# MaaniGhaffari/cvo-rgbd

Hardware: AMD Instinct MI355X
Metric: frame-pair registrations/sec (higher is better)
Workload: dtype f32; 1 GPU; BASELINE configs[1] shape: 64 distinct synthetic 10000x10000 RGB-D cloud pairs (xyz + 5-dim colour) per align_many call, cvo align() to convergence, clouds resident in HBM; points_fixed=10000, points_moving=10000, mode=cvo, batch=64

## Files before the change

cvo-rgbd_amd/capi.py:

```python
import collections
import ctypes as C
import os

import numpy as np

_HERE = os.path.dirname(os.path.abspath(__file__))
LIB_PATH = os.path.join(_HERE, "csrc", "libcvo_hip.so")
_LIB = None

MODE_CVO, MODE_ACVO, MODE_MATLAB = 0, 1, 2
FEAT_COLMAJOR, FEAT_ROWMAJOR = 0, 1

SYMBOLS = [
    "cvo_hip_error_string", "cvo_hip_last_error", "cvo_hip_device_count",
    "cvo_hip_default_params", "cvo_hip_init_state", "cvo_hip_create", "cvo_hip_destroy",
    "cvo_hip_set_params", "cvo_hip_set_fixed", "cvo_hip_set_moving",
    "cvo_hip_set_fixed_device", "cvo_hip_set_moving_device",
    "cvo_hip_swap_moving_to_fixed", "cvo_hip_set_pcd_many", "cvo_hip_get_device_cloud", "cvo_hip_range_filter_grid_average", "cvo_hip_set_shard", "cvo_hip_shard_range",
    "cvo_hip_comm_unique_id", "cvo_hip_comm_init", "cvo_hip_set_allreduce",
    "cvo_hip_mailbox_create", "cvo_hip_mailbox_connect",
    "cvo_hip_transform_pcd", "cvo_hip_flow", "cvo_hip_step_coeffs", "cvo_hip_pose_hessian", "cvo_hip_pose_score",
    "cvo_hip_pose_score_many", "cvo_hip_pose_scan", "cvo_hip_pose_matches", "cvo_hip_pick_step",
    "cvo_hip_exp_se3", "cvo_hip_dist_se3", "cvo_hip_align", "cvo_hip_align_many",
    "cvo_hip_function_inner_product", "cvo_hip_function_inner_product_clouds",
    "cvo_hip_engine_profiling", "cvo_hip_get_engine_profile", "cvo_hip_get_engine_flow_trace", "cvo_hip_get_wave_load", "cvo_hip_set_graph_capture", "cvo_hip_set_profiling", "cvo_hip_get_profile", "cvo_hip_get_graph_stats", "cvo_hip_get_run_stats", "cvo_hip_get_list_stats", "cvo_hip_get_run_clocks", "cvo_hip_get_mirror_retries", "cvo_hip_synchronize",
    "cvo_hip_set_option", "cvo_hip_get_option",
]


class Params(C.Structure):
    _fields_ = [
        ("mode", C.c_int32), ("max_iter", C.c_int32),
        ("ell_init", C.c_float), ("ell_min", C.c_float), ("ell_max_init", C.c_float),
        ("sigma", C.c_float), ("sp_thres", C.c_float), ("c_sp_thres", C.c_float),
        ("c", C.c_float), ("d", C.c_float), ("c_ell", C.c_float), ("c_sigma", C.c_float),
        ("min_step", C.c_float), ("eps", C.c_float), ("eps_2", C.c_float), ("color_scale", C.c_float),
        ("dl_step", C.c_double),
    ]


class State(C.Structure):
    _fields_ = [
        ("R", C.c_float * 9), ("T", C.c_float * 3),
        ("ell", C.c_float), ("ell_max", C.c_float),
        ("transform", C.c_float * 16), ("prev_transform", C.c_float * 16),
        ("accum_transform", C.c_float * 16),
        ("iter", C.c_int32), ("pad_", C.c_int32),
    ]
# ... 150 lines not shown
    L.cvo_hip_transform_pcd.argtypes = [vp, fp, fp]
    L.cvo_hip_flow.argtypes = [vp, C.c_float, dp]
    L.cvo_hip_step_coeffs.argtypes = [vp, fp, fp, C.c_float, dp]
    L.cvo_hip_pose_hessian.argtypes = [vp, fp, fp, C.c_float, C.POINTER(PoseHessianC)]
    L.cvo_hip_pose_score.argtypes = [vp, fp, fp, C.c_float, C.POINTER(PoseScoreC)]
    L.cvo_hip_pose_score_many.argtypes = [C.POINTER(vp), fp, fp, fp, C.POINTER(PoseScoreC), C.c_int]
    L.cvo_hip_pose_scan.argtypes = [vp, fp, fp, C.c_int, C.c_float, C.POINTER(PoseScanEntryC), C.POINTER(PoseScanC)]
    L.cvo_hip_pose_matches.argtypes = [vp, fp, fp, C.c_float, C.POINTER(PointMatchesC), C.POINTER(PointMatchesC),
                                       C.POINTER(PoseMatchesC)]
    L.cvo_hip_pick_step.argtypes = [dp, C.c_float, fp]
    L.cvo_hip_exp_se3.argtypes = [fp, fp, C.c_float, fp, fp]
    L.cvo_hip_dist_se3.argtypes = [fp, fp, C.c_float, fp]
    L.cvo_hip_align.argtypes = [vp, C.POINTER(State), C.POINTER(Trace), C.c_int,
                                C.POINTER(C.c_int)]
    L.cvo_hip_align_many.argtypes = [C.POINTER(vp), C.POINTER(C.POINTER(State)), C.POINTER(C.c_int),
                                     C.c_int]
    L.cvo_hip_function_inner_product.argtypes = [vp, C.c_float, fp]
    L.cvo_hip_function_inner_product_clouds.argtypes = [vp, C.c_float, fp, fp, C.c_int, fp, fp, C.c_int,
                                                        C.c_int, fp]
    L.cvo_hip_engine_profiling.argtypes = [C.c_int]
    L.cvo_hip_get_engine_profile.argtypes = [dp, C.POINTER(C.c_longlong), dp, C.c_int]
    L.cvo_hip_get_engine_flow_trace.argtypes = [fp, fp, C.POINTER(C.c_int), C.c_int, C.POINTER(C.c_int), C.c_int]
    L.cvo_hip_get_wave_load.argtypes = [vp, C.POINTER(C.c_uint32), C.c_int, C.POINTER(C.c_int)]
    L.cvo_hip_set_graph_capture.argtypes = [vp, C.c_int]
    L.cvo_hip_set_profiling.argtypes = [vp, C.c_int]
    L.cvo_hip_get_profile.argtypes = [vp, C.POINTER(Profile), C.c_int]
    L.cvo_hip_get_graph_stats.argtypes = [vp, C.POINTER(C.c_longlong), C.POINTER(C.c_longlong)]
    L.cvo_hip_get_run_clocks.argtypes = [vp, C.POINTER(C.c_longlong)]
    L.cvo_hip_get_mirror_retries.argtypes = []
    L.cvo_hip_get_mirror_retries.restype = C.c_longlong
    L.cvo_hip_get_run_stats.argtypes = [vp, C.POINTER(C.c_int), C.POINTER(C.c_int), C.POINTER(C.c_int), C.POINTER(C.c_int)]
    L.cvo_hip_get_list_stats.argtypes = [vp, C.POINTER(C.c_int), C.POINTER(C.c_int), C.POINTER(C.c_int)]
    L.cvo_hip_synchronize.argtypes = [vp]
    L.cvo_hip_set_option.argtypes = [vp, C.c_char_p, C.c_double]
    L.cvo_hip_get_option.argtypes = [vp, C.c_char_p, C.POINTER(C.c_double)]
    for name in SYMBOLS:
        if name not in ("cvo_hip_error_string", "cvo_hip_last_error"):
            getattr(L, name).restype = C.c_int
    _LIB = L
    return L


def check(status, ctx=None, what=""):
    if status == 0:
        return
    L = lib()
# ... 274 lines not shown
        self._chk(self._L.cvo_hip_align(self._ctx, C.byref(state), tr, trace_cap, C.byref(n_it)),
                  "align")
        n = n_it.value
        return n, [trace_to_dict(tr[i]) for i in range(min(n, trace_cap))]

    def function_inner_product(self, ell):
        out = C.c_float()
        self._chk(self._L.cvo_hip_function_inner_product(self._ctx, np.float32(ell), C.byref(out)),
                  "function_inner_product")
        return out.value

    def function_inner_product_clouds(self, ell, xyz_a, feat_a, xyz_b, feat_b, layout=FEAT_ROWMAJOR):
        xyz_a, feat_a, xyz_b, feat_b = f32(xyz_a), f32(feat_a), f32(xyz_b), f32(feat_b)
        out = C.c_float()
        self._chk(self._L.cvo_hip_function_inner_product_clouds(
            self._ctx, np.float32(ell), fptr(xyz_a), fptr(feat_a), xyz_a.shape[0], fptr(xyz_b), fptr(feat_b),
            xyz_b.shape[0], layout, C.byref(out)), "function_inner_product_clouds")
        return out.value

    def wave_load(self):
        buf = (C.c_uint32 * 4096)()
        n = C.c_int(0)
        self._chk(self._L.cvo_hip_get_wave_load(self._ctx, buf, 4096, C.byref(n)), "wave_load")
        return np.array(buf[:n.value], np.int64)

    def set_profiling(self, enable=True):
        self._chk(self._L.cvo_hip_set_profiling(self._ctx, int(bool(enable))), "set_profiling")

    def get_profile(self, reset=False):
        p = Profile()
        self._chk(self._L.cvo_hip_get_profile(self._ctx, C.byref(p), int(reset)), "get_profile")
        return {k: getattr(p, k) for k, _ in Profile._fields_}

    def graph_stats(self):
        a, b = C.c_longlong(0), C.c_longlong(0)
        self._chk(self._L.cvo_hip_get_graph_stats(self._ctx, C.byref(a), C.byref(b)), "graph_stats")
        return a.value, b.value

    def run_stats(self):
        a, b, c, d = C.c_int(0), C.c_int(0), C.c_int(0), C.c_int(0)
        self._chk(self._L.cvo_hip_get_run_stats(self._ctx, C.byref(a), C.byref(b), C.byref(c), C.byref(d)), "run_stats")
        return a.value, b.value, c.value, d.value

    def list_stats(self):
        a, b, c = C.c_int(0), C.c_int(0), C.c_int(0)
        self._chk(self._L.cvo_hip_get_list_stats(self._ctx, C.byref(a), C.byref(b), C.byref(c)), "list_stats")
# ... 116 lines not shown
```

cvo-rgbd_amd/csrc/cvo_capi.cpp:

```cpp
#include "cvo_internal.h"

using namespace cvo_dev;
using namespace cvo_impl;

namespace cvo_impl {

int fail(cvo_hip_ctx *ctx, int code, const char *msg)
{
    if (ctx) ctx->err = msg;
    return code;
}

static std::atomic<bool> g_engine_debug{false};
bool engine_debug_on() { return g_engine_debug.load(std::memory_order_relaxed); }

namespace {
struct OptDef {
    const char *key;
    const char *env;
    int env_kind;
    double env_value;
};
const OptDef kOptions[] = {
    {"graph_capture", "CVO_HIP_GRAPH", 1, 1.0},           {"no_graph", "CVO_HIP_NO_GRAPH", 1, 1.0},
// ... 682 lines not shown
    HIP_TRY(ctx, hipSetDevice(ctx->device));
    const bool had_tf = ctx->have_tf;
    std::swap(ctx->fixed, ctx->scratch_a);
    std::swap(ctx->moving, ctx->scratch_b);
    int rc = upload_cloud(ctx, ctx->fixed, xyz_a, feat_a, na, feat_layout);
    if (!rc) rc = upload_cloud(ctx, ctx->moving, xyz_b, feat_b, nb, feat_layout);
    if (!rc) rc = cvo_hip_function_inner_product(ctx, ell, out);
    std::swap(ctx->fixed, ctx->scratch_a);
    std::swap(ctx->moving, ctx->scratch_b);
    ctx->have_tf = had_tf;
    return rc;
}

int cvo_hip_get_wave_load(cvo_hip_ctx *ctx, uint32_t *members_per_wave, int capacity, int *waves)
{
    cvo_lock::Api api_guard;
    if (!ctx || !members_per_wave || !waves || capacity < 0) return CVO_HIP_ERR_INVALID;
    HIP_TRY(ctx, hipSetDevice(ctx->device));
    const int n = std::min(capacity, 4 * ctx->proc_blocks);
    *waves = 0;
    if (!ctx->kept_cnt.p || n <= 0) return CVO_HIP_OK;
    HIP_TRY(ctx, hipStreamSynchronize(ctx->stream));
    HIP_TRY(ctx, hipMemcpy(members_per_wave, ctx->kept_cnt.p, (size_t)n * sizeof(uint32_t), hipMemcpyDeviceToHost));
    *waves = n;
    return CVO_HIP_OK;
}

int cvo_hip_set_graph_capture(cvo_hip_ctx *ctx, int enable)
{
    cvo_lock::Api api_guard;
    if (!ctx) return CVO_HIP_ERR_INVALID;
    return apply_option(ctx, "graph_capture", enable ? 1.0 : 0.0);
}

int cvo_hip_set_profiling(cvo_hip_ctx *ctx, int enable)
{
    cvo_lock::Api api_guard;
    if (!ctx) return CVO_HIP_ERR_INVALID;
    ctx->profiling = enable != 0;
    return CVO_HIP_OK;
}

int cvo_hip_get_profile(cvo_hip_ctx *ctx, cvo_hip_profile *out, int reset)
{
    cvo_lock::Api api_guard;
    if (!ctx || !out) return CVO_HIP_ERR_INVALID;
// ... 138 lines not shown
```

cvo-rgbd_amd/csrc/cvo_device.h:

```cpp
#pragma once

#include <hip/hip_runtime.h>
#include <hip/hip_ext.h>
#include <stddef.h>
#include <stdint.h>

#include "cvo_hip.h"
#include "se3_math.hpp"

namespace cvo_dev {

constexpr int FEAT_STRIDE = 8;
constexpr int FEAT_INDEX_SLOT = 5;

constexpr int BLOCK = 256;
constexpr int TILES_PER_WAVE = 4;
constexpr int ROWS_PER_WAVE = 16 * TILES_PER_WAVE;
constexpr int ROWS_PER_TILE = 4 * ROWS_PER_WAVE;
constexpr float PAD_BIG = 1.0e30f;
constexpr int PROC_BLOCKS = 1024;
constexpr int PROC_WAVES = PROC_BLOCKS * 4;

constexpr int NSUB = 256;
constexpr int PROC_PARTS = PROC_BLOCKS / NSUB;
constexpr int TILE_STAGE = 128;
constexpr int DEAL_SHIFT = 2;
constexpr int PAIR_QUEUE = 128;
constexpr int SEG = 64;
constexpr int MAX_CSEG = 32;

typedef uint4 TileEntry;

enum ProcMode { PROC_FLOW = 0, PROC_STEP = 1, PROC_SELF = 2 };
enum ListId { LIST_XY = 0, LIST_XX = 1, LIST_YY = 2, LIST_KEPT = 3, LIST_XYB = 4, LIST_XXB = 5, LIST_YYB = 6,
              LIST_N = 7 };
CVO_HD int self_list_id(int l, int buf) { return buf ? LIST_XXB + l : LIST_XX + l; }

constexpr int NACC_FLOW = 9;
constexpr int NACC_STEP = 4;
constexpr int NACC_SELF = 2;
constexpr int NACC_MAX = 9;

constexpr int RED_FLOW = 0, RED_XX = 9, RED_YY = 11, RED_STEP = 13, RED_N = 17;

enum { RUNNING = 0, DONE_BREAK_A = 1, DONE_BREAK_B = 2, DONE_MAX_ITER = 3, NEED_BIGGER_LIST = 4,
       DONE_COMM_ERROR = 5,
       DONE_RUN_TIMEOUT = 6 };

constexpr int MAX_WORLD = 16;
constexpr int MAIL_VALS = 14;
struct alignas(128) MailSlot {
    double v[MAIL_VALS];
    unsigned long long seq;
    unsigned long long pad_;
};
struct Mailbox {
    MailSlot slot[2][MAX_WORLD];
    unsigned long long owner_dev;
    unsigned long long pad_[15];
// ... 620 lines not shown
{
    return *reinterpret_cast<const float4 *>(static_cast<const char *>(base) + byte_off);
}
template <bool W>
__device__ __forceinline__ float4 load_pos(const CVO_GLOBAL char *base, unsigned byte_off)
{
    if (W) {
        const f32x4_t v = *reinterpret_cast<const CVO_GLOBAL f32x4_t *>(base + byte_off);
        return make_float4(v.x, v.y, v.z, v.w);
    }
    typedef float f32x3_t __attribute__((ext_vector_type(3)));
    const f32x3_t v = *reinterpret_cast<const CVO_GLOBAL f32x3_t *>(base + byte_off);
    return make_float4(v.x, v.y, v.z, 0.0f);
}
__device__ __forceinline__ uint2 load8(const CVO_GLOBAL char *base, unsigned idx)
{
#ifdef CVO_NT_LISTS
    const u32x2_t v = __builtin_nontemporal_load(reinterpret_cast<const CVO_GLOBAL u32x2_t *>(base) + idx);
#else
    const u32x2_t v = reinterpret_cast<const CVO_GLOBAL u32x2_t *>(base)[idx];
#endif
    return make_uint2(v.x, v.y);
}
__device__ __forceinline__ uint2 kept_pack(const int mode, const unsigned ebase, const unsigned i, const unsigned j, const float w)
{
    if (mode == 1) return make_uint2(i | (j << 16), __float_as_uint(w));
    const unsigned wb = __float_as_uint(w);
    return make_uint2(i | (j << 18), (j >> 14) | (((wb >> 23) - ebase) << 4) | ((wb & 0x7fffffu) << 8));
}
__device__ __forceinline__ void kept_unpack(const int mode, const unsigned ebase, const uint2 e, const float raw_w, unsigned &i,
                                            unsigned &j, float &w)
{
    if (mode == 0) { i = e.x; j = e.y; w = raw_w; }
    else if (mode == 1) { i = e.x & 0xffffu; j = e.x >> 16; w = __uint_as_float(e.y); }
    else {
        i = e.x & 0x3ffffu;
        j = (e.x >> 18) | ((e.y & 0xfu) << 14);
        w = __uint_as_float(((((e.y >> 4) & 0xfu) + ebase) << 23) | ((e.y >> 8) & 0x7fffffu));
    }
}
__device__ __forceinline__ const CVO_GLOBAL char *kept_slice(const KeptView &k, const int wid, size_t &base, unsigned &n)
{
    const unsigned wave = blockIdx.x * 4u + (unsigned)wid;
    base = (size_t)wave * k.kept_wcap;
    n = k.kept_cnt[wave];
    if (n > k.kept_wcap) n = k.kept_wcap;
// ... 222 lines not shown
```

cvo-rgbd_amd/csrc/cvo_kernels.hip:

```cpp
#include <algorithm>
#include <atomic>
#include <cstdlib>

#include "cvo_device.h"
#include "cvo_pair.h"

namespace cvo_dev {

typedef float f32x4 __attribute__((ext_vector_type(4)));

__device__ __forceinline__ float mv_row(const float *m, float x, float y, float z)
{
    return (m[0] * x + m[1] * y) + m[2] * z;
}

constexpr int FILTER_KMAX = 64;
size_t filter_smem_bytes(int jt)
{
    return (size_t)jt * 16 + ROWS_PER_TILE * 16 + 4 * TILE_STAGE * sizeof(TileEntry) +
           FILTER_KMAX * 4 * 4;
}

__device__ __forceinline__ void flush_tiles(const TileEntry *stage, int n, int lane, unsigned rot, unsigned region,
                                            const FilterArgs &a, int list, TileEntry *tiles, const int par)
// ... 534 lines not shown
    }
    const f32x2 normxiz2 = (xiz[0] * xiz[0] + xiz[1] * xiz[1]) + xiz[2] * xiz[2];
    const f32x2 xz12 = -((xiz[0] * xi2z[0] + xiz[1] * xi2z[1]) + xiz[2] * xi2z[2]);
    const f32x2 eps_c = ((xi2z[0] * xi2z[0] + xi2z[1] * xi2z[1]) + xi2z[2] * xi2z[2]) +
                        2.0f * ((xiz[0] * xi3z[0] + xiz[1] * xi3z[1]) + xiz[2] * xi3z[2]);
    const float cb = kc.cb, cg = kc.cg, cd = kc.cd;
    const f32x2 beta = ((cb * xiz[0]) * e0 + (cb * xiz[1]) * e1) + (cb * xiz[2]) * e2;
    const f32x2 g_dot = ((2.0f * xi2z[0]) * e0 + (2.0f * xi2z[1]) * e1) + (2.0f * xi2z[2]) * e2;
    const f32x2 gamma = cg * (normxiz2 + g_dot);
    const f32x2 d_dot = ((-xi3z[0]) * e0 + (-xi3z[1]) * e1) + (-xi3z[2]) * e2;
    const f32x2 delta = cd * (xz12 + d_dot);
    const f32x2 e_dot = ((2.0f * xi4z[0]) * e0 + (2.0f * xi4z[1]) * e1) + (2.0f * xi4z[2]) * e2;
    const f32x2 epsil = cg * (eps_c + e_dot);
    step_tail(w.x, beta.x, gamma.x, delta.x, epsil.x, acc);
    step_tail(w.y, beta.y, gamma.y, delta.y, epsil.y, acc);
}

template <int MODE, int WEIGHT = 0, int CK = 0, class ARGS = ProcessArgs>
__device__ __forceinline__ float eval_pair(const ARGS &a, const ProcHead &hd, const KernConsts &kc, unsigned i,
                                           unsigned j, float w, double *acc,
                                           const cvo_math::XiConsts &xc, const double *etab = nullptr,
                                           const int first_counted = 0, float *ck_io = nullptr,
                                           uint2 *pf_out = nullptr, const CVO_GLOBAL char *pf_base = nullptr, unsigned pf_idx = 0,
                                           float *d2_out = nullptr )
{
    const float *Rt = hd.Rt;
    const float *tt = hd.tt;
    constexpr bool need_w = MODE != PROC_STEP && CK != 2;
    float4 xi = load_pos<need_w>(a.pos_a, i * 16u);
    float4 yj = load_pos<need_w>(a.pos_b, j * 16u);
    if (pf_out) *pf_out = load8(pf_base, pf_idx);
    float4 fa0 = make_float4(0.f, 0.f, 0.f, 0.f), fb0 = fa0;
    float fa4 = 0.f, fb4 = 0.f;
    int row_index = 0;
    if (MODE != PROC_STEP && CK != 2) {
        fa0 = *gather16(a.feat_a, i * (unsigned)(FEAT_STRIDE * 4));
        fb0 = *gather16(a.feat_b, j * (unsigned)(FEAT_STRIDE * 4));
        fa4 = xi.w;
        fb4 = yj.w;
        if (MODE == PROC_SELF)
            row_index = __float_as_int(a.feat_a[(size_t)i * FEAT_STRIDE + FEAT_INDEX_SLOT]);
    }
    if (a.tf_a) xi = apply_tf(Rt, tt, xi);
    if (a.tf_b) yj = apply_tf(Rt, tt, yj);
    const float e0 = xi.x - yj.x, e1 = xi.y - yj.y, e2 = xi.z - yj.z;
    float d2 = 0.0f;
    if (MODE != PROC_STEP) {
        d2 = __builtin_fmaf(e2, e2, __builtin_fmaf(e1, e1, e0 * e0));
        if (d2_out) *d2_out = d2;
        if (CK == 0) {
            w = (d2 < kc.tau) ? pair_weight<WEIGHT>(kc, d2, fa0, fa4, fb0, fb4, etab) : 0.0f;
        } else {
            const float ck = CK == 2 ? __builtin_fabsf(*ck_io) : colour_weight(kc, fa0, fa4, fb0, fb4, etab);
            if (CK == 2 && MODE == PROC_SELF) row_index = (*ck_io < 0.0f) ? -1 : 0;
// ... 83 lines not shown
        int qn = 0;
        unsigned nk = 0;
        unsigned co = 0;
        const size_t kbase = (size_t)wave * a.kept_wcap;
        auto run_batch = [&](int base, int cnt) {
            __builtin_amdgcn_fence(__ATOMIC_RELEASE, "wavefront");
            __builtin_amdgcn_wave_barrier();
            __builtin_amdgcn_fence(__ATOMIC_ACQUIRE, "wavefront");
            float w = 0.0f;
            uint2 pr = make_uint2(0u, 0u);
            float ck = 0.0f;
            float d2 = 0.0f;
            if (lane < cnt) {
                pr = pairq[base + lane];
                w = eval_pair<MODE, WEIGHT, REC>(src, hd, kc, pr.x, pr.y, 0.0f, acc, *hd.xi, s_etab, first_counted, &ck,
                                                 nullptr, nullptr, 0, (REC && MODE == PROC_FLOW) ? &d2 : nullptr);
            }
            if (REC && MODE == PROC_FLOW) {
                const unsigned long long cm = __ballot(lane < cnt && !(d2 >= hd.rec_lim));
                const unsigned add = (unsigned)__popcll(cm);
                if (co + add <= a.kept_wcap) {
                    if (lane < cnt && !(d2 >= hd.rec_lim)) {
                        const unsigned below = __builtin_amdgcn_mbcnt_hi((unsigned)(cm >> 32), __builtin_amdgcn_mbcnt_lo((unsigned)cm, 0u));
                        hd.cand[kbase + co + below] = make_uint2(pr.x | (pr.y << 16), __float_as_uint(ck));
                    }
                } else if (lane == 0) {
                    atomicOr(&a.st->ovf[hd.par][LIST_KEPT], 1u);
                }
                co += add;
            } else if (REC) {
                if (co + (unsigned)cnt <= a.kept_wcap) {
                    if (lane < cnt) hd.cand[kbase + co + lane] = make_uint2(pr.x | (pr.y << 16), __float_as_uint(ck));
                } else if (lane == 0) {
                    atomicOr(&a.st->ovf[hd.par][LIST_KEPT], 1u);
                }
                co += (unsigned)cnt;
            }
            if (MODE == PROC_SELF) nk += (unsigned)__popcll(__ballot(w > 0.0f));
            if (MODE == PROC_FLOW) {
                const unsigned long long km = __ballot(w > 0.0f);
                const unsigned add = (unsigned)__popcll(km);
                if (nk + add <= a.kept_wcap) {
#ifndef CVO_PROBE_NO_KEPT_STORE
                    if (w > 0.0f) {
#else
                    if (false) {
#endif
                        const unsigned below = __builtin_amdgcn_mbcnt_hi(
                            (unsigned)(km >> 32), __builtin_amdgcn_mbcnt_lo((unsigned)km, 0u));
                        if (a.kept_packed) {
                            a.kept_ij[kbase + nk + below] = kept_pack(a.kept_packed, a.kept_ebase, pr.x, pr.y, w);
                        } else {
                            a.kept_ij[kbase + nk + below] = pr;
                            a.kept_a[kbase + nk + below] = w;
                        }
// ... 36 lines not shown
                const unsigned r = ty >> 30, tcol = ty & 0x3fffffffu;
                if (__builtin_amdgcn_inverse_ballot_w64(m)) {
                    const unsigned below = __builtin_amdgcn_mbcnt_hi(
                        (unsigned)(m >> 32), __builtin_amdgcn_mbcnt_lo((unsigned)m, 0u));
                    pairq[qn + below] =
                        make_uint2(tx + (unsigned)(lane >> 4) * 4u + r, tcol + (unsigned)(lane & 15));
                }
                qn += __popcll(m);
                if (qn >= 64) {
                    qn -= 64;
                    run_batch(qn, 64);
                }
            }
        }
        sub += (unsigned)a.nblk; n = n_next; tl = tl_next; mine = mine_next;
        }
        if (qn > 0) run_batch(0, qn);
        if (MODE == PROC_FLOW && lane == 0) a.kept_cnt[wave] = nk;
        if (REC && lane == 0) hd.cand_cnt[wave] = co;
        if (lane == 0) acc[MODE == PROC_FLOW ? 8 : 1] = (double)nk;
        return true;
}

template <int MODE, bool PIPE, bool NARROW = false>
__device__ __forceinline__ bool stream_candidates(const ProcessArgs &a, const ProcHead &hd, const KernConsts &kc, const int lane,
                                                  const unsigned wave, const int done_word, const double *s_etab,
                                                  double (&acc)[NAcc<MODE>::n])
{
    unsigned wcap = a.kept_wcap;
    const size_t base = (size_t)wave * wcap;
    unsigned n = hd.cand_cnt[wave];
    uint2 e = list_load(&hd.cand[base + lane]);
    if (done_word != 0) return false;
    if (n > wcap) n = wcap;
    unsigned nk = 0;
    unsigned co = 0;
    const PairSrc src = pin_pair_src<PIPE>(a);
    const CVO_GLOBAL char *cand_w = pin_global<PIPE>(hd.cand + base);
    const CVO_GLOBAL char *kept_w = pin_global<PIPE>(a.kept_ij + base);
    wcap = pin_u32<PIPE>(wcap);
    constexpr bool PF = PIPE && kPrefetchBuild;
    for (unsigned b0 = 0; b0 < n; b0 += 64u) {
        if (!PF && b0 != 0u) e = load8(cand_w, min(b0 + (unsigned)lane, wcap - 1u));
        uint2 e_next = e;
        uint2 *const pf = PF ? &e_next : nullptr;
        const unsigned ci = e.x & 0xffffu, cj = e.x >> 16;
        float w = 0.0f;
        float d2 = PAD_BIG;
        if (b0 + (unsigned)lane < n) {
            float ck = __uint_as_float(e.y);
            w = eval_pair<MODE, 0, 2>(src, hd, kc, ci, cj, 0.0f, acc, *hd.xi, s_etab, 0, &ck, pf, cand_w,
                                      min(b0 + 64u + (unsigned)lane, wcap - 1u), NARROW ? &d2 : nullptr);
        }
        if (NARROW && PF) asm volatile("" : "+v"(e_next.x), "+v"(e_next.y));
        if (NARROW) {
            const unsigned long long cm = __ballot(d2 < hd.rec_lim);
            if (d2 < hd.rec_lim) {
                const unsigned below = __builtin_amdgcn_mbcnt_hi((unsigned)(cm >> 32), __builtin_amdgcn_mbcnt_lo((unsigned)cm, 0u));
                store8(cand_w, co + below, e.x, e.y);
            }
            co += (unsigned)__popcll(cm);
        }
        const unsigned long long km = __ballot(w > 0.0f);
        if (MODE == PROC_FLOW && w > 0.0f) {
            const unsigned below = __builtin_amdgcn_mbcnt_hi((unsigned)(km >> 32), __builtin_amdgcn_mbcnt_lo((unsigned)km, 0u));
#ifndef CVO_PROBE_NO_KEPT_STORE
            store8(kept_w, nk + below, e.x, __float_as_uint(w));
#endif
        }
        nk += (unsigned)__popcll(km);
        if (PF) e = e_next;
    }
    if (lane == 0) {
#if defined(CVO_PROBE_NO_KEPT_STORE) || defined(CVO_PROBE_KEPT_CNT0)
        if (MODE == PROC_FLOW) a.kept_cnt[wave] = 0u;
#else
        if (MODE == PROC_FLOW) a.kept_cnt[wave] = nk;
#endif
        acc[MODE == PROC_FLOW ? 8 : 1] = (double)nk;
        if (NARROW) hd.cand_cnt[wave] = co;
    }
    return true;
}

template <int MODE, int WEIGHT = 0, bool CAND = true, bool PIPE = true>
__device__ __forceinline__ void process_body(const ProcessArgs &a, const unsigned bid, char *scratch, const ProcHead &hd)
{
    if ((int)bid >= a.nblk) return;
    constexpr int NACC = NAcc<MODE>::n;
    double *red = reinterpret_cast<double *>(scratch);
    uint2 *pairq_all = reinterpret_cast<uint2 *>(scratch + 4 * NACC_MAX * 8);
    double *s_etab_all = reinterpret_cast<double *>(scratch + 4 * NACC_MAX * 8 + 4 * PAIR_QUEUE * 8);
#ifdef CVO_PROBE_STEP_EXP
    s_etab_all[threadIdx.x] = c_exp2_64[threadIdx.x & 63];
// ... 1877 lines not shown
    float cx[NRX][3], cy[NRX][3], cck[NRX], cw[NRX];
    float4 *const lc = s_lc + tid;
    auto load_xy = [&]() {
    const unsigned total = tot_cur;
    const int act = act_cur;
    const unsigned wave_first = head_block ? total : (unsigned)srow * RUN_BLOCK + (unsigned)wid * 64u;
    rmax = wave_first < total ? (int)((total - wave_first + lanes - 1) / lanes) : 0;
    {
        const uint2 *rec = act ? pa.cand_b : pa.cand;
        const unsigned wcap = pa.kept_wcap;
        uint2 e[NRX];
#pragma unroll
        for (int r = 0; r < NRX; ++r) {
            e[r] = make_uint2(0u, 0u);
            if (r < rmax) {
                const unsigned c0 = wave_first + (unsigned)r * lanes;
                const unsigned coarse = s_pref[lane * 64];
                const int k1 = __popcll(__ballot(coarse <= c0)) - 1;
                const unsigned fine = s_pref[k1 * 64 + lane];
                int sl = k1 * 64 + __popcll(__ballot(fine <= c0)) - 1;
                const unsigned c = c0 + (unsigned)lane;
                if (c < total) {
                    while (c >= s_pref[sl + 1]) ++sl;
                    e[r] = rec[(size_t)sl * wcap + (c - s_pref[sl])];
                }
            }
        }
#pragma unroll
        for (int r = 0; r < NRX; ++r) {
            cck[r] = 0.0f; cw[r] = 0.0f;
            cx[r][0] = cx[r][1] = cx[r][2] = 0.0f;
            cy[r][0] = cy[r][1] = cy[r][2] = 0.0f;
            if (r < rmax) {
                const bool have = wave_first + (unsigned)r * lanes + (unsigned)lane < total;
                const float4 x = pa.pos_a[e[r].x & 0xffffu];
                const float4 y = pa.pos_b[e[r].x >> 16];
                cx[r][0] = x.x; cx[r][1] = x.y; cx[r][2] = x.z;
                cy[r][0] = y.x; cy[r][1] = y.y; cy[r][2] = y.z;
                cck[r] = have ? __uint_as_float(e[r].y) : 0.0f;
            }
        }
    }
    static_assert(RUN_L % 2 == 0, "run_flow_lds / run_step_lds take two rounds per trip");
    nl = (!ACVO && rmax > RUN_R) ? ((rmax - RUN_R + 1) & ~1) : 0;
    {
        const uint2 *rec = act ? pa.cand_b : pa.cand;
        const unsigned wcap = pa.kept_wcap;
#pragma unroll 1
        for (int r0 = 0; r0 < nl; r0 += 2) {
            uint2 e[2];
            bool have[2];
#pragma unroll
            for (int u = 0; u < 2; ++u) {
                const unsigned c0 = wave_first + (unsigned)(RUN_R + r0 + u) * lanes;
                const unsigned cs = c0 < total ? c0 : total - 1u;
                const unsigned coarse = s_pref[lane * 64];
                const int k1 = __popcll(__ballot(coarse <= cs)) - 1;
                const unsigned fine = s_pref[k1 * 64 + lane];
                int sl = k1 * 64 + __popcll(__ballot(fine <= cs)) - 1;
                const unsigned c = c0 + (unsigned)lane;
                e[u] = make_uint2(0u, 0u);
                have[u] = c < total;
                if (have[u]) {
                    while (c >= s_pref[sl + 1]) ++sl;
                    e[u] = rec[(size_t)sl * wcap + (c - s_pref[sl])];
                }
            }
            float4 x[2], y[2];
#pragma unroll
            for (int u = 0; u < 2; ++u) { x[u] = pa.pos_a[e[u].x & 0xffffu]; y[u] = pa.pos_b[e[u].x >> 16]; }
#pragma unroll
            for (int u = 0; u < 2; ++u) {
                lc[(2 * (r0 + u)) * RUN_BLOCK] = make_float4(x[u].x, x[u].y, x[u].z, have[u] ? __uint_as_float(e[u].y) : 0.0f);
                lc[(2 * (r0 + u) + 1) * RUN_BLOCK] = make_float4(y[u].x, y[u].y, y[u].z, 0.0f);
            }
        }
    }
    };
    load_xy();
    float xd2[ACVO ? RUN_A : 1], xck[ACVO ? RUN_A : 1];
    float yya[ACVO ? RUN_A : 1][3], yyb[ACVO ? RUN_A : 1][3], yck[ACVO ? RUN_A : 1];
    int rmax_x = 0, rmax_y = 0;
    if constexpr (ACVO) {
#pragma unroll
        for (int set = 0; set < 2; ++set) {
            const ProcessArgs &sa = set == 0 ? xa : ya;
            const unsigned tot_s = set == 0 ? total_x : total_y;
            const uint2 *rec = (set == 0 ? act_x : act_y) ? sa.cand_b : sa.cand;
            const unsigned wcap = sa.kept_wcap;
            const unsigned *const pref = s_pref_self + (set == 0 ? 0 : PROC_WAVES + 1);
            const unsigned first_s = head_block ? tot_s : (unsigned)srow * RUN_BLOCK + (unsigned)wid * 64u;
            const int rm = first_s < tot_s ? (int)((tot_s - first_s + lanes - 1) / lanes) : 0;
            if (set == 0) rmax_x = rm; else rmax_y = rm;
            uint2 e[RUN_A];
#pragma unroll
            for (int r = 0; r < RUN_A; ++r) {
                e[r] = make_uint2(0u, 0u);
                if (r < rm) {
                    const unsigned c0 = first_s + (unsigned)r * lanes;
                    const unsigned coarse = pref[lane * 64];
                    const int k1 = __popcll(__ballot(coarse <= c0)) - 1;
                    const unsigned fine = pref[k1 * 64 + lane];
                    int sl = k1 * 64 + __popcll(__ballot(fine <= c0)) - 1;
                    const unsigned c = c0 + (unsigned)lane;
                    if (c < tot_s) {
                        while (c >= pref[sl + 1]) ++sl;
                        e[r] = rec[(size_t)sl * wcap + (c - pref[sl])];
                    }
                }
            }
#pragma unroll
            for (int r = 0; r < RUN_A; ++r) {
                const bool have = r < rm && first_s + (unsigned)r * lanes + (unsigned)lane < tot_s;
                const float4 a4 = sa.pos_a[e[r].x & 0xffffu];
                const float4 b4 = sa.pos_b[e[r].x >> 16];
                const float ckr = have ? __uint_as_float(e[r].y) : 0.0f;
                if (set == 0) {
                    const float e0 = a4.x - b4.x, e1 = a4.y - b4.y, e2 = a4.z - b4.z;
                    xd2[r] = __builtin_fmaf(e2, e2, __builtin_fmaf(e1, e1, e0 * e0));
                    xck[r] = ckr;
                } else {
                    yya[r][0] = a4.x; yya[r][1] = a4.y; yya[r][2] = a4.z;
                    yyb[r][0] = b4.x; yyb[r][1] = b4.y; yyb[r][2] = b4.z;
                    yck[r] = ckr;
                }
            }
        }
        if (tid == 0) { s_xx_ell = -1.0f; s_xx_keep[0] = 0.0; s_xx_keep[1] = 0.0; }
        __syncthreads();
    }
// ... 525 lines not shown
```

cvo-rgbd_amd/csrc/cvo_plan.cpp:

```cpp
#include "cvo_internal.h"

using namespace cvo_dev;
using namespace cvo_impl;

namespace cvo_impl {

FilterPlan plan_filter(int nrows, int nb)
{
    FilterPlan p{};
    const int tiles = std::max(1, (nrows + ROWS_PER_TILE - 1) / ROWS_PER_TILE);
    const int want_blocks = 4096;
    const int chunks_want = std::max(1, (want_blocks + tiles / 2) / tiles);
    int jt = (nb + chunks_want - 1) / chunks_want;
    jt = std::max(jt, 64);
    jt = std::min(jt, 2048);
    jt = (jt + SEG - 1) & ~(SEG - 1);
    p.jt = jt;
    const int chunks = std::max(1, (nb + jt - 1) / jt);
    p.grid = dim3(chunks, tiles);
    return p;
}

int ensure_buf(cvo_hip_ctx *ctx, DevBuf &b, size_t bytes)
{
    if (bytes <= b.bytes) return CVO_HIP_OK;
    if (b.p) HIP_TRY(ctx, hipFree(b.p));
    b.p = nullptr;
    b.bytes = 0;
    if (hipMalloc(&b.p, bytes) != hipSuccess) {
        b.p = nullptr;
        return fail(ctx, CVO_HIP_ERR_NOMEM, "hipMalloc failed (candidate list / partials)");
    }
    b.bytes = bytes;
    return CVO_HIP_OK;
}

int ensure_list(cvo_hip_ctx *ctx, int list, int nrows, int nb, double at_least)
{
    List &L = ctx->lists[list];
    double want;
    uint32_t min_sub;
    if (list == LIST_KEPT) {
        const double all = (double)std::max(nrows, 0) * (double)std::max(nb, 0);
        want = std::max(all * 0.04, 1048576.0);
        want = std::min(want, std::max(all * 1.25, 1.0));
        min_sub = 64 * (PROC_WAVES / NSUB);
    } else {
        const double all = std::ceil(std::max(nrows, 0) / 16.0 + 1.0) * std::ceil(std::max(nb, 0) / 16.0 + 1.0);
        want = (all * 4.0 * sizeof(TileEntry) <= 64.0e6) ? all * 4.0 : std::max(all * 0.25, 64.0e6 / sizeof(TileEntry));
        min_sub = TILE_STAGE;
    }
    if (at_least <= 0.0) {
        if (ctx->opt.list_init > 0.0) want = ctx->opt.list_init;
    }
    want = std::max(want, at_least);
    want = std::min(want, 4.0e9);
    const uint32_t cap = std::max<uint32_t>((uint32_t)((want + NSUB - 1) / NSUB), min_sub) * NSUB;
    if (cap <= L.cap) return CVO_HIP_OK;
    int rc;
    if (list == LIST_KEPT) {
        rc = ensure_buf(ctx, L.a, (size_t)cap * sizeof(uint2));
        if (!rc) rc = ensure_buf(ctx, L.b, (size_t)cap * sizeof(float));
    } else {
        rc = ensure_buf(ctx, L.a, (size_t)cap * sizeof(TileEntry));
    }
    if (rc) return rc;
    L.cap = cap;
    return CVO_HIP_OK;
}
// ... 123 lines not shown
    if (!no_pack && ctx->fixed.np <= 65536 && ctx->moving.np <= 65536) return 1;
    if (!no_pack && weight == 0 && ctx->fixed.np <= 262144 && ctx->moving.np <= 262144) {
        const float amax = (float)ctx->dprm.cs2_d * (float)ctx->dprm.s2_d;
        uint32_t blo, bhi;
        std::memcpy(&blo, &ctx->dprm.sp, sizeof(blo));
        std::memcpy(&bhi, &amax, sizeof(bhi));
        const uint32_t elo = blo >> 23, ehi = bhi >> 23;
        if (ctx->dprm.sp > 0.0f && amax > ctx->dprm.sp && elo >= 1 && ehi < 255 && ehi - elo <= 15) {
            *ebase = elo;
            return 2;
        }
    }
    return 0;
}

KeptView kept_view(const cvo_hip_ctx *ctx)
{
    KeptView v{};
    v.kept_ij = (const uint2 *)ctx->lists[LIST_KEPT].a.p;
    v.kept_a = (const float *)ctx->lists[LIST_KEPT].b.p;
    v.kept_cnt = (const uint32_t *)ctx->kept_cnt.p;
    v.st = ctx->st;
    v.nblk = ctx->proc_blocks;
    v.kept_wcap = ctx->lists[LIST_KEPT].cap / (uint32_t)(4 * ctx->proc_blocks);
    v.kept_packed = kept_format(ctx, &v.kept_ebase);
    return v;
}

int enqueue_process(cvo_hip_ctx *ctx, int mode, int list, DevBuf &part, const float4 *pos_a,
                    const float *feat_a, int tf_a, const float4 *pos_b, const float *feat_b,
                    int tf_b, int first_counted, int check_done)
{
    int rc = ensure_buf(ctx, part, (size_t)PROC_WAVES * NACC_MAX * sizeof(double));
    if (rc) return rc;
    rc = ensure_list(ctx, list, 0, 0, 0);
    if (rc) return rc;
    if (!ctx->kept_cnt.p) {
        rc = ensure_buf(ctx, ctx->kept_cnt, PROC_WAVES * sizeof(uint32_t));
        if (rc) return rc;
        HIP_TRY(ctx, hipMemsetAsync(ctx->kept_cnt.p, 0, PROC_WAVES * sizeof(uint32_t), ctx->stream));
    }
    if (mode == PROC_FLOW)
        rc = ensure_list(ctx, LIST_KEPT, ctx->fixed.np, ctx->moving.np, 0);
    else
        rc = ensure_list(ctx, LIST_KEPT, 0, 0, 0);
    if (rc) return rc;
    ProcessArgs a{};
    a.pos_a = pos_a; a.feat_a = feat_a;
    a.pos_b = pos_b; a.feat_b = feat_b;
    a.tiles = (const TileEntry *)ctx->lists[list].a.p;
    a.kept_ij = (uint2 *)ctx->lists[LIST_KEPT].a.p;
    a.kept_a = (float *)ctx->lists[LIST_KEPT].b.p;
    a.kept_cnt = (uint32_t *)ctx->kept_cnt.p;
    a.partials = (double *)part.p;
    a.st = ctx->st;
    a.st2 = static_cast<DevState *>(ctx->st2);
    a.subcap = ctx->lists[list].cap / NSUB;
    a.nblk = ctx->proc_blocks;
    a.kept_wcap = ctx->lists[LIST_KEPT].cap / (uint32_t)(4 * ctx->proc_blocks);
    a.list = list;
    a.first_counted = first_counted;
    a.tf_a = tf_a; a.tf_b = tf_b;
    if (pre_transform(ctx) && ctx->pos_bt.p) {
        if (tf_b && pos_b == ctx->moving.pos) { a.pos_b = (const float4 *)ctx->pos_bt.p; a.tf_b = 0; }
        if (tf_a && pos_a == ctx->moving.pos) { a.pos_a = (const float4 *)ctx->pos_bt.p; a.tf_a = 0; }
    }
    a.check_done = check_done;
    a.need_d2 = (ctx->prm.mode == CVO_HIP_MODE_ACVO || !ctx->in_loop || ctx->cur_trace_cap > 0) ? 1 : 0;
    a.weight = ctx->prm.color_scale > 0.0f ? 1 : 0;
    a.kept_packed = kept_format(ctx, &a.kept_ebase);
    if ((mode == PROC_FLOW && list == LIST_XY) || (mode == PROC_SELF && (list == LIST_XX || list == LIST_YY))) {
        const bool no_cand = ctx->opt.no_cand;
        ctx->ck_nblk[list] = 0;
        if (!no_cand && pre_transform(ctx) && !(ctx->prm.color_scale > 0.0f) && a.kept_packed == 1) {
            int rc_c = ensure_buf(ctx, ctx->cand[list], (size_t)ctx->lists[LIST_KEPT].cap * sizeof(uint2));
            if (!rc_c) rc_c = ensure_buf(ctx, ctx->cand_cnt[list], PROC_WAVES * sizeof(uint32_t));
            if (!rc_c) {
                a.cand = (uint2 *)ctx->cand[list].p;
                a.cand_cnt = (uint32_t *)ctx->cand_cnt[list].p;
                ctx->ck_nblk[list] = a.nblk;
            } else {
                (void)hipGetLastError();
// ... 841 lines not shown
```

include/cvo_hip.h:

```cpp
#ifndef CVO_HIP_H
#define CVO_HIP_H

#include <stdint.h>

#ifdef __cplusplus
extern "C" {
#endif

#define CVO_HIP_NFEAT 5

typedef enum cvo_hip_status {
    CVO_HIP_OK = 0,
    CVO_HIP_ERR_INVALID = -1,
    CVO_HIP_ERR_HIP = -2,
    CVO_HIP_ERR_NOMEM = -3,
    CVO_HIP_ERR_COMM = -4,
    CVO_HIP_ERR_NODEVICE = -5,
    CVO_HIP_ERR_RUN = -6
} cvo_hip_status;

enum { CVO_HIP_MODE_CVO = 0, CVO_HIP_MODE_ACVO = 1, CVO_HIP_MODE_MATLAB = 2 };
enum { CVO_HIP_FEAT_COLMAJOR = 0, CVO_HIP_FEAT_ROWMAJOR = 1 };

typedef struct cvo_hip_params {
// ... 190 lines not shown
int cvo_hip_align(cvo_hip_ctx *ctx, cvo_hip_state *state, cvo_hip_trace *trace,
                  int trace_cap, int *n_iter);

int cvo_hip_align_many(cvo_hip_ctx **ctxs, cvo_hip_state **states, int *n_iters, int count);

int cvo_hip_function_inner_product(cvo_hip_ctx *ctx, float ell, float *out);
int cvo_hip_function_inner_product_clouds(cvo_hip_ctx *ctx, float ell, const float *xyz_a,
                                          const float *feat_a, int na, const float *xyz_b,
                                          const float *feat_b, int nb, int feat_layout, float *out);

int cvo_hip_set_graph_capture(cvo_hip_ctx *ctx, int enable);

int cvo_hip_set_option(cvo_hip_ctx *ctx, const char *key, double value);
int cvo_hip_get_option(const cvo_hip_ctx *ctx, const char *key, double *value);

int cvo_hip_set_profiling(cvo_hip_ctx *ctx, int enable);
int cvo_hip_get_profile(cvo_hip_ctx *ctx, cvo_hip_profile *out, int reset);

int cvo_hip_engine_profiling(int enable);
int cvo_hip_get_engine_profile(double *flow_ms, long long *flow_launches, double *flow_registrations, int reset);
int cvo_hip_get_engine_flow_trace(float *dur_us, float *period_us, int *slots, int capacity, int *count, int reset);

int cvo_hip_get_wave_load(cvo_hip_ctx *ctx, uint32_t *members_per_wave, int capacity, int *waves);

int cvo_hip_get_graph_stats(const cvo_hip_ctx *ctx, long long *launches_from_cache, long long *captures);
int cvo_hip_get_run_stats(cvo_hip_ctx *ctx, int *runs, int *declined, int *iterations, int *candidates);
int cvo_hip_get_list_stats(const cvo_hip_ctx *ctx, int *builds, int *narrowings, int *reexpansions);
int cvo_hip_get_run_clocks(cvo_hip_ctx *ctx, long long clocks16[16]);
long long cvo_hip_get_mirror_retries(void);
int cvo_hip_synchronize(cvo_hip_ctx *ctx);

#ifdef __cplusplus
}
#endif
#endif
```

Before: 4427 registrations/s.

## Interleave candidate records in 128-entry blocks for 16-byte paired loads

Candidate records are now stored in an interleaved order inside 128-entry blocks, so each lane reads two records with a single 16-byte load and processes them in two rounds. The streaming loop is split out into a stream_round helper, and per-wave capacity is rounded down to a multiple of the block size. Readers in the downstream kernels are updated to the same permuted index. The aim is fewer, wider memory transactions when streaming candidates, at the cost of slightly reduced per-wave capacity, extra index arithmetic and higher register pressure. A debugging API for reading record load is also added.

```diff
diff --git a/cvo-rgbd_amd/capi.py b/cvo-rgbd_amd/capi.py
--- a/cvo-rgbd_amd/capi.py
+++ b/cvo-rgbd_amd/capi.py
@@ -23,7 +23,7 @@
     "cvo_hip_pose_score_many", "cvo_hip_pose_scan", "cvo_hip_pose_matches", "cvo_hip_pick_step",
     "cvo_hip_exp_se3", "cvo_hip_dist_se3", "cvo_hip_align", "cvo_hip_align_many",
     "cvo_hip_function_inner_product", "cvo_hip_function_inner_product_clouds",
-    "cvo_hip_engine_profiling", "cvo_hip_get_engine_profile", "cvo_hip_get_engine_flow_trace", "cvo_hip_get_wave_load", "cvo_hip_set_graph_capture", "cvo_hip_set_profiling", "cvo_hip_get_profile", "cvo_hip_get_graph_stats", "cvo_hip_get_run_stats", "cvo_hip_get_list_stats", "cvo_hip_get_run_clocks", "cvo_hip_get_mirror_retries", "cvo_hip_synchronize",
+    "cvo_hip_engine_profiling", "cvo_hip_get_engine_profile", "cvo_hip_get_engine_flow_trace", "cvo_hip_get_wave_load", "cvo_hip_get_record_load", "cvo_hip_set_graph_capture", "cvo_hip_set_profiling", "cvo_hip_get_profile", "cvo_hip_get_graph_stats", "cvo_hip_get_run_stats", "cvo_hip_get_list_stats", "cvo_hip_get_run_clocks", "cvo_hip_get_mirror_retries", "cvo_hip_synchronize",
     "cvo_hip_set_option", "cvo_hip_get_option",
 ]
 
@@ -220,6 +220,7 @@
     L.cvo_hip_get_engine_profile.argtypes = [dp, C.POINTER(C.c_longlong), dp, C.c_int]
     L.cvo_hip_get_engine_flow_trace.argtypes = [fp, fp, C.POINTER(C.c_int), C.c_int, C.POINTER(C.c_int), C.c_int]
     L.cvo_hip_get_wave_load.argtypes = [vp, C.POINTER(C.c_uint32), C.c_int, C.POINTER(C.c_int)]
+    L.cvo_hip_get_record_load.argtypes = [vp, C.c_int, C.POINTER(C.c_uint32), C.c_int, C.POINTER(C.c_int)]
     L.cvo_hip_set_graph_capture.argtypes = [vp, C.c_int]
     L.cvo_hip_set_profiling.argtypes = [vp, C.c_int]
     L.cvo_hip_get_profile.argtypes = [vp, C.POINTER(Profile), C.c_int]
@@ -540,6 +541,12 @@
         buf = (C.c_uint32 * 4096)()
         n = C.c_int(0)
         self._chk(self._L.cvo_hip_get_wave_load(self._ctx, buf, 4096, C.byref(n)), "wave_load")
+        return np.array(buf[:n.value], np.int64)
+
+    def record_load(self, buffer=0):
+        buf = (C.c_uint32 * 4096)()
+        n = C.c_int(0)
+        self._chk(self._L.cvo_hip_get_record_load(self._ctx, int(buffer), buf, 4096, C.byref(n)), "record_load")
         return np.array(buf[:n.value], np.int64)
 
     def set_profiling(self, enable=True):
diff --git a/cvo-rgbd_amd/csrc/cvo_capi.cpp b/cvo-rgbd_amd/csrc/cvo_capi.cpp
--- a/cvo-rgbd_amd/csrc/cvo_capi.cpp
+++ b/cvo-rgbd_amd/csrc/cvo_capi.cpp
@@ -728,6 +728,26 @@
     if (!ctx->kept_cnt.p || n <= 0) return CVO_HIP_OK;
     HIP_TRY(ctx, hipStreamSynchronize(ctx->stream));
     HIP_TRY(ctx, hipMemcpy(members_per_wave, ctx->kept_cnt.p, (size_t)n * sizeof(uint32_t), hipMemcpyDeviceToHost));
+    *waves = n;
+    return CVO_HIP_OK;
+}
+
+int cvo_hip_get_record_load(cvo_hip_ctx *ctx, int buffer, uint32_t *candidates_per_wave, int capacity, int *waves)
+{
+    cvo_lock::Api api_guard;
+    if (!ctx || !candidates_per_wave || !waves || capacity < 0 || buffer < 0 || buffer > 1) return CVO_HIP_ERR_INVALID;
+    HIP_TRY(ctx, hipSetDevice(ctx->device));
+    const DevBuf &cnt = buffer ? ctx->cand_cnt_xyb : ctx->cand_cnt[LIST_XY];
+    *waves = 0;
+    if (!cnt.p || !ctx->st) return CVO_HIP_OK;
+    HIP_TRY(ctx, hipStreamSynchronize(ctx->stream));
+    int32_t ck = 0, xy_ck[2] = {0, 0};
+    HIP_TRY(ctx, hipMemcpy(&ck, reinterpret_cast<const char *>(ctx->st) + offsetof(DevState, ck_nblk) + LIST_XY * sizeof(int32_t), sizeof(ck), hipMemcpyDeviceToHost));
+    HIP_TRY(ctx, hipMemcpy(xy_ck, reinterpret_cast<const char *>(ctx->st) + offsetof(DevState, xy_ck), sizeof(xy_ck), hipMemcpyDeviceToHost));
+    const int nblk = buffer ? xy_ck[1] : (ck ? ck : xy_ck[0]);
+    const int n = std::min(capacity, 4 * std::min(std::max(nblk, 0), (int)PROC_BLOCKS));
+    if (n <= 0) return CVO_HIP_OK;
+    HIP_TRY(ctx, hipMemcpy(candidates_per_wave, cnt.p, (size_t)n * sizeof(uint32_t), hipMemcpyDeviceToHost));
     *waves = n;
     return CVO_HIP_OK;
 }
diff --git a/cvo-rgbd_amd/csrc/cvo_device.h b/cvo-rgbd_amd/csrc/cvo_device.h
--- a/cvo-rgbd_amd/csrc/cvo_device.h
+++ b/cvo-rgbd_amd/csrc/cvo_device.h
@@ -35,6 +35,18 @@
 enum ListId { LIST_XY = 0, LIST_XX = 1, LIST_YY = 2, LIST_KEPT = 3, LIST_XYB = 4, LIST_XXB = 5, LIST_YYB = 6,
               LIST_N = 7 };
 CVO_HD int self_list_id(int l, int buf) { return buf ? LIST_XXB + l : LIST_XX + l; }
+
+constexpr unsigned REC_BLOCK = 128;
+#ifdef CVO_LINEAR_REC
+constexpr bool kPairedRec = false;
+#else
+constexpr bool kPairedRec = true;
+#endif
+CVO_HD unsigned cand_pos(unsigned k)
+{
+    return kPairedRec ? (k & ~(REC_BLOCK - 1u)) + ((k & 63u) << 1) + ((k >> 6) & 1u) : k;
+}
+CVO_HD uint32_t rec_wcap(uint32_t cap, uint32_t waves) { return (cap / waves) & ~(REC_BLOCK - 1u); }
 
 constexpr int NACC_FLOW = 9;
 constexpr int NACC_STEP = 4;
@@ -701,6 +713,16 @@
 #endif
     return make_uint2(v.x, v.y);
 }
+__device__ __forceinline__ uint4 load16(const CVO_GLOBAL char *base, unsigned idx)
+{
+    typedef unsigned u32x4_t __attribute__((ext_vector_type(4)));
+#ifdef CVO_NT_LISTS
+    const u32x4_t v = __builtin_nontemporal_load(reinterpret_cast<const CVO_GLOBAL u32x4_t *>(base + idx * 8u));
+#else
+    const u32x4_t v = *reinterpret_cast<const CVO_GLOBAL u32x4_t *>(base + idx * 8u);
+#endif
+    return make_uint4(v.x, v.y, v.z, v.w);
+}
 __device__ __forceinline__ uint2 kept_pack(const int mode, const unsigned ebase, const unsigned i, const unsigned j, const float w)
 {
     if (mode == 1) return make_uint2(i | (j << 16), __float_as_uint(w));
diff --git a/cvo-rgbd_amd/csrc/cvo_kernels.hip b/cvo-rgbd_amd/csrc/cvo_kernels.hip
--- a/cvo-rgbd_amd/csrc/cvo_kernels.hip
+++ b/cvo-rgbd_amd/csrc/cvo_kernels.hip
@@ -580,7 +580,8 @@
                                            const cvo_math::XiConsts &xc, const double *etab = nullptr,
                                            const int first_counted = 0, float *ck_io = nullptr,
                                            uint2 *pf_out = nullptr, const CVO_GLOBAL char *pf_base = nullptr, unsigned pf_idx = 0,
-                                           float *d2_out = nullptr )
+                                           float *d2_out = nullptr ,
+                                           uint4 *pf16_out = nullptr )
 {
     const float *Rt = hd.Rt;
     const float *tt = hd.tt;
@@ -588,6 +589,7 @@
     float4 xi = load_pos<need_w>(a.pos_a, i * 16u);
     float4 yj = load_pos<need_w>(a.pos_b, j * 16u);
     if (pf_out) *pf_out = load8(pf_base, pf_idx);
+    if (pf16_out) *pf16_out = load16(pf_base, pf_idx);
     float4 fa0 = make_float4(0.f, 0.f, 0.f, 0.f), fb0 = fa0;
     float fa4 = 0.f, fb4 = 0.f;
     int row_index = 0;
@@ -717,7 +719,7 @@
                 if (co + add <= a.kept_wcap) {
                     if (lane < cnt && !(d2 >= hd.rec_lim)) {
                         const unsigned below = __builtin_amdgcn_mbcnt_hi((unsigned)(cm >> 32), __builtin_amdgcn_mbcnt_lo((unsigned)cm, 0u));
-                        hd.cand[kbase + co + below] = make_uint2(pr.x | (pr.y << 16), __float_as_uint(ck));
+                        hd.cand[kbase + cand_pos(co + below)] = make_uint2(pr.x | (pr.y << 16), __float_as_uint(ck));
                     }
                 } else if (lane == 0) {
                     atomicOr(&a.st->ovf[hd.par][LIST_KEPT], 1u);
@@ -725,7 +727,7 @@
                 co += add;
             } else if (REC) {
                 if (co + (unsigned)cnt <= a.kept_wcap) {
-                    if (lane < cnt) hd.cand[kbase + co + lane] = make_uint2(pr.x | (pr.y << 16), __float_as_uint(ck));
+                    if (lane < cnt) hd.cand[kbase + cand_pos(co + (unsigned)lane)] = make_uint2(pr.x | (pr.y << 16), __float_as_uint(ck));
                 } else if (lane == 0) {
                     atomicOr(&a.st->ovf[hd.par][LIST_KEPT], 1u);
                 }
@@ -808,6 +810,40 @@
         return true;
 }
 
+template <int MODE, bool NARROW, int PFW, int NACC>
+__device__ __forceinline__ void stream_round(const PairSrc &src, const ProcHead &hd, const KernConsts &kc, const double *s_etab,
+                                             double (&acc)[NACC], const CVO_GLOBAL char *cand_w, const CVO_GLOBAL char *kept_w,
+                                             const unsigned ex, const unsigned ey, const bool have, const unsigned pf_idx,
+                                             uint2 &e8_next, uint4 &e16_next, unsigned &nk, unsigned &co)
+{
+    const unsigned ci = ex & 0xffffu, cj = ex >> 16;
+    float w = 0.0f;
+    float d2 = PAD_BIG;
+    if (have) {
+        float ck = __uint_as_float(ey);
+        w = eval_pair<MODE, 0, 2>(src, hd, kc, ci, cj, 0.0f, acc, *hd.xi, s_etab, 0, &ck, PFW == 1 ? &e8_next : nullptr, cand_w, pf_idx,
+                                  NARROW ? &d2 : nullptr, PFW == 2 ? &e16_next : nullptr);
+    }
+    if (NARROW && PFW == 1) asm volatile("" : "+v"(e8_next.x), "+v"(e8_next.y));
+    if (NARROW && PFW == 2) asm volatile("" : "+v"(e16_next.x), "+v"(e16_next.y), "+v"(e16_next.z), "+v"(e16_next.w));
+    if (NARROW) {
+        const unsigned long long cm = __ballot(d2 < hd.rec_lim);
+        if (d2 < hd.rec_lim) {
+            const unsigned below = __builtin_amdgcn_mbcnt_hi((unsigned)(cm >> 32), __builtin_amdgcn_mbcnt_lo((unsigned)cm, 0u));
+            store8(cand_w, cand_pos(co + below), ex, ey);
+        }
+        co += (unsigned)__popcll(cm);
+    }
+    const unsigned long long km = __ballot(w > 0.0f);
+    if (MODE == PROC_FLOW && w > 0.0f) {
+        const unsigned below = __builtin_amdgcn_mbcnt_hi((unsigned)(km >> 32), __builtin_amdgcn_mbcnt_lo((unsigned)km, 0u));
+#ifndef CVO_PROBE_NO_KEPT_STORE
+        store8(kept_w, nk + below, ex, __float_as_uint(w));
+#endif
+    }
+    nk += (unsigned)__popcll(km);
+}
+
 template <int MODE, bool PIPE, bool NARROW = false>
 __device__ __forceinline__ bool stream_candidates(const ProcessArgs &a, const ProcHead &hd, const KernConsts &kc, const int lane,
                                                   const unsigned wave, const int done_word, const double *s_etab,
@@ -816,7 +852,10 @@
     unsigned wcap = a.kept_wcap;
     const size_t base = (size_t)wave * wcap;
     unsigned n = hd.cand_cnt[wave];
-    uint2 e = list_load(&hd.cand[base + lane]);
+    uint2 e = make_uint2(0u, 0u);
+    uint4 e4 = make_uint4(0u, 0u, 0u, 0u);
+    if (kPairedRec) e4 = load16((const CVO_GLOBAL char *)(unsigned long long)(hd.cand + base), 2u * (unsigned)lane);
+    else e = list_load(&hd.cand[base + lane]);
     if (done_word != 0) return false;
     if (n > wcap) n = wcap;
     unsigned nk = 0;
@@ -826,36 +865,24 @@
     const CVO_GLOBAL char *kept_w = pin_global<PIPE>(a.kept_ij + base);
     wcap = pin_u32<PIPE>(wcap);
     constexpr bool PF = PIPE && kPrefetchBuild;
-    for (unsigned b0 = 0; b0 < n; b0 += 64u) {
-        if (!PF && b0 != 0u) e = load8(cand_w, min(b0 + (unsigned)lane, wcap - 1u));
-        uint2 e_next = e;
-        uint2 *const pf = PF ? &e_next : nullptr;
-        const unsigned ci = e.x & 0xffffu, cj = e.x >> 16;
-        float w = 0.0f;
-        float d2 = PAD_BIG;
-        if (b0 + (unsigned)lane < n) {
-            float ck = __uint_as_float(e.y);
-            w = eval_pair<MODE, 0, 2>(src, hd, kc, ci, cj, 0.0f, acc, *hd.xi, s_etab, 0, &ck, pf, cand_w,
-                                      min(b0 + 64u + (unsigned)lane, wcap - 1u), NARROW ? &d2 : nullptr);
-        }
-        if (NARROW && PF) asm volatile("" : "+v"(e_next.x), "+v"(e_next.y));
-        if (NARROW) {
-            const unsigned long long cm = __ballot(d2 < hd.rec_lim);
-            if (d2 < hd.rec_lim) {
-                const unsigned below = __builtin_amdgcn_mbcnt_hi((unsigned)(cm >> 32), __builtin_amdgcn_mbcnt_lo((unsigned)cm, 0u));
-                store8(cand_w, co + below, e.x, e.y);
-            }
-            co += (unsigned)__popcll(cm);
-        }
-        const unsigned long long km = __ballot(w > 0.0f);
-        if (MODE == PROC_FLOW && w > 0.0f) {
-            const unsigned below = __builtin_amdgcn_mbcnt_hi((unsigned)(km >> 32), __builtin_amdgcn_mbcnt_lo((unsigned)km, 0u));
-#ifndef CVO_PROBE_NO_KEPT_STORE
-            store8(kept_w, nk + below, e.x, __float_as_uint(w));
-#endif
-        }
-        nk += (unsigned)__popcll(km);
-        if (PF) e = e_next;
+    if (kPairedRec) {
+        for (unsigned b0 = 0; b0 < n; b0 += REC_BLOCK) {
+            if (!PF && b0 != 0u) e4 = load16(cand_w, b0 + 2u * (unsigned)lane);
+            uint4 e4_next = e4;
+            stream_round<MODE, NARROW, 0>(src, hd, kc, s_etab, acc, cand_w, kept_w, e4.x, e4.y, b0 + (unsigned)lane < n, 0u, e, e4_next, nk, co);
+            if (b0 + 64u < n)
+                stream_round<MODE, NARROW, PF ? 2 : 0>(src, hd, kc, s_etab, acc, cand_w, kept_w, e4.z, e4.w, b0 + 64u + (unsigned)lane < n,
+                                                       min(b0 + REC_BLOCK + 2u * (unsigned)lane, wcap - 2u), e, e4_next, nk, co);
+            if (PF) e4 = e4_next;
+        }
+    } else {
+        for (unsigned b0 = 0; b0 < n; b0 += 64u) {
+            if (!PF && b0 != 0u) e = load8(cand_w, min(b0 + (unsigned)lane, wcap - 1u));
+            uint2 e_next = e;
+            stream_round<MODE, NARROW, PF ? 1 : 0>(src, hd, kc, s_etab, acc, cand_w, kept_w, e.x, e.y, b0 + (unsigned)lane < n,
+                                                   min(b0 + 64u + (unsigned)lane, wcap - 1u), e_next, e4, nk, co);
+            if (PF) e = e_next;
+        }
     }
     if (lane == 0) {
 #if defined(CVO_PROBE_NO_KEPT_STORE) || defined(CVO_PROBE_KEPT_CNT0)
@@ -2779,7 +2806,7 @@
                 const unsigned c = c0 + (unsigned)lane;
                 if (c < total) {
                     while (c >= s_pref[sl + 1]) ++sl;
-                    e[r] = rec[(size_t)sl * wcap + (c - s_pref[sl])];
+                    e[r] = rec[(size_t)sl * wcap + cand_pos(c - s_pref[sl])];
                 }
             }
         }
@@ -2820,7 +2847,7 @@
                 have[u] = c < total;
                 if (have[u]) {
                     while (c >= s_pref[sl + 1]) ++sl;
-                    e[u] = rec[(size_t)sl * wcap + (c - s_pref[sl])];
+                    e[u] = rec[(size_t)sl * wcap + cand_pos(c - s_pref[sl])];
                 }
             }
             float4 x[2], y[2];
@@ -2862,7 +2889,7 @@
                     const unsigned c = c0 + (unsigned)lane;
                     if (c < tot_s) {
                         while (c >= pref[sl + 1]) ++sl;
-                        e[r] = rec[(size_t)sl * wcap + (c - pref[sl])];
+                        e[r] = rec[(size_t)sl * wcap + cand_pos(c - pref[sl])];
                     }
                 }
             }
diff --git a/cvo-rgbd_amd/csrc/cvo_plan.cpp b/cvo-rgbd_amd/csrc/cvo_plan.cpp
--- a/cvo-rgbd_amd/csrc/cvo_plan.cpp
+++ b/cvo-rgbd_amd/csrc/cvo_plan.cpp
@@ -44,7 +44,7 @@
         const double all = (double)std::max(nrows, 0) * (double)std::max(nb, 0);
         want = std::max(all * 0.04, 1048576.0);
         want = std::min(want, std::max(all * 1.25, 1.0));
-        min_sub = 64 * (PROC_WAVES / NSUB);
+        min_sub = REC_BLOCK * (PROC_WAVES / NSUB);
     } else {
         const double all = std::ceil(std::max(nrows, 0) / 16.0 + 1.0) * std::ceil(std::max(nb, 0) / 16.0 + 1.0);
         want = (all * 4.0 * sizeof(TileEntry) <= 64.0e6) ? all * 4.0 : std::max(all * 0.25, 64.0e6 / sizeof(TileEntry));
@@ -214,7 +214,7 @@
     v.kept_cnt = (const uint32_t *)ctx->kept_cnt.p;
     v.st = ctx->st;
     v.nblk = ctx->proc_blocks;
-    v.kept_wcap = ctx->lists[LIST_KEPT].cap / (uint32_t)(4 * ctx->proc_blocks);
+    v.kept_wcap = rec_wcap(ctx->lists[LIST_KEPT].cap, (uint32_t)(4 * ctx->proc_blocks));
     v.kept_packed = kept_format(ctx, &v.kept_ebase);
     return v;
 }
@@ -249,7 +249,7 @@
     a.st2 = static_cast<DevState *>(ctx->st2);
     a.subcap = ctx->lists[list].cap / NSUB;
     a.nblk = ctx->proc_blocks;
-    a.kept_wcap = ctx->lists[LIST_KEPT].cap / (uint32_t)(4 * ctx->proc_blocks);
+    a.kept_wcap = rec_wcap(ctx->lists[LIST_KEPT].cap, (uint32_t)(4 * ctx->proc_blocks));
     a.list = list;
     a.first_counted = first_counted;
     a.tf_a = tf_a; a.tf_b = tf_b;
diff --git a/include/cvo_hip.h b/include/cvo_hip.h
--- a/include/cvo_hip.h
+++ b/include/cvo_hip.h
@@ -236,6 +236,7 @@
 int cvo_hip_get_engine_flow_trace(float *dur_us, float *period_us, int *slots, int capacity, int *count, int reset);
 
 int cvo_hip_get_wave_load(cvo_hip_ctx *ctx, uint32_t *members_per_wave, int capacity, int *waves);
+int cvo_hip_get_record_load(cvo_hip_ctx *ctx, int buffer, uint32_t *candidates_per_wave, int capacity, int *waves);
 
 int cvo_hip_get_graph_stats(const cvo_hip_ctx *ctx, long long *launches_from_cache, long long *captures);
 int cvo_hip_get_run_stats(cvo_hip_ctx *ctx, int *runs, int *declined, int *iterations, int *candidates);
```

Measured after the change: 4471 registrations/s, median of 6. No clear change (+1.0%).
